# HorizonRobotics/HoloAgent

Hardware: AMD Instinct MI355X
Metric: HMSG frames/sec (one scene per GPU: map A1-A2, fusion A3-A5, merge A6, pooling A7, floors A8, rooms by the device watershed N1, room clouds, room embeddings and View nodes A9, objects with the view <-> object test A10 and graph assembly A11, nothing handed in -- plus 1000 coarse-to-fine retrieval qu (higher is better)
Workload: dtype f64 geometry / f32 features

## Files before the change

### holoagent_amd/csrc/hmsg_api.hip

```cpp
#include "hmsg_boundary.h"
#include "hmsg_ckdtree.h"
#include "hmsg_nn.h"
#include "hmsg_rle.h"

#include <algorithm>
#include <cstring>
#include <stdexcept>

void hmsg_bitset(hmsg_ctx* h, int first, int n, int M, const unsigned char* d_masks, const int* d_nmask);
void hmsg_fp_tables(hmsg_ctx* h, int first, int n, int M, const float* d_fg, const float* d_fm, const float* d_fc, const int* d_nmask);

__global__ void k_nn_patch(const long long* __restrict__ qid, const int* __restrict__ val, unsigned n, int* __restrict__ target) {
    const unsigned i = blockIdx.x * blockDim.x + threadIdx.x;
    if (i < n) target[qid[i]] = val[i];
}

void hmsg_kd_join(hmsg_ctx* h) {
    if (h->kd_thread.joinable()) h->kd_thread.join();
}

void hmsg_kd_start(hmsg_ctx* h) {
    hmsg_kd_join(h);
    h->host_pts.resize((size_t)h->V * 3);
    if (h->V) HIP_TRY(hipMemcpyAsync(h->host_pts.data(), h->pts.p, (size_t)h->V * 24, hipMemcpyDeviceToHost, h->stream));
// ... 129 lines not shown
        HIP_TRY(hipSetDevice(cfg->device_id));
        HIP_TRY(hipStreamCreateWithFlags(&h->stream, hipStreamNonBlocking));
        alloc_frame_store(h);
        h->pose.alloc((size_t)16 * cfg->max_frames);
    });
    if (rc != HMSG_OK) {
        delete h;
        return rc;
    }
    *out = h;
    return HMSG_OK;
}

void hmsg_destroy(hmsg_t* h) {
    if (!h) return;
    hmsg_kd_join(h);
    (void)hipSetDevice(h->cfg.device_id);
    try {
        hmsg_fold_pipe_abort(h);
    } catch (...) {
    }
    hmsg_graph_early_abort(h);
    h->fold_cache.trim();
    if (h->stream) {
        (void)hipStreamSynchronize(h->stream);
        (void)hipStreamDestroy(h->stream);
    }
    delete h;
}

const char* hmsg_last_error(const hmsg_t* h) { return h ? h->err.c_str() : "null handle"; }

void hmsg_release_cached_memory(void) { dev_cache().trim(); }

int hmsg_reset(hmsg_t* h) {
    if (!h) return HMSG_ERR_INVALID;
    return hmsg_boundary(h, [&] {
        HIP_TRY(hipStreamSynchronize(h->stream));
        hmsg_kd_join(h);
        hmsg_fold_pipe_abort(h);
        hmsg_graph_early_abort(h);
        ++h->inst_epoch;
        h->n_tie_queries = 0;
        h->n_frames = h->n_feat_frames = h->n_fused = 0;
        h->n_offered = 0;
        h->room_n = 0;
// ... 528 lines not shown
```

### holoagent_amd/csrc/hmsg_common.h

```cpp
#pragma once
#include <hip/hip_runtime.h>

#include <algorithm>
#include <chrono>
#include <cstdarg>
#include <cstdint>
#include <cstdio>
#include <cstdlib>
#include <cstring>
#include <map>
#include <memory>
#include <mutex>
#include <thread>
#include <string>
#include <vector>

#include "../../include/hmsg.h"
#include "../../include/hmsg_test.h"

#define HMSG_WAVE 64

struct hmsg_error {
    int code;
    std::string msg;
// ... 232 lines not shown
    ScopedEvent() { HIP_TRY(hipEventCreate(&e)); }
    ScopedEvent(const ScopedEvent&) = delete;
    ScopedEvent& operator=(const ScopedEvent&) = delete;
    ~ScopedEvent() { (void)hipEventDestroy(e); }
    operator hipEvent_t() const { return e; }
};

template <typename T>
struct PinnedBuf {
    T* p = nullptr;
    size_t n = 0;
    PinnedBuf() = default;
    PinnedBuf(const PinnedBuf&) = delete;
    PinnedBuf& operator=(const PinnedBuf&) = delete;
    ~PinnedBuf() {
        if (p) (void)hipHostFree(p);
    }
    void ensure(size_t count) {
        if (count <= n) return;
        if (p) (void)hipHostFree(p);
        p = nullptr;
        n = std::max<size_t>(count * 2, 256);
        HIP_TRY(hipHostMalloc((void**)&p, n * sizeof(T), hipHostMallocDefault));
    }
};
inline void d2h_bounce(void* dst, const void* src, size_t bytes) {
    constexpr size_t CH = (size_t)16 << 20;
    if (bytes <= 4096) {
        HIP_TRY(hipMemcpy(dst, src, bytes, hipMemcpyDeviceToHost));
        return;
    }
    static std::mutex mu;
    static PinnedBuf<unsigned char> stage;
    std::lock_guard<std::mutex> lk(mu);
    stage.ensure(std::min(bytes, CH));
    for (size_t o = 0; o < bytes; o += CH) {
        const size_t n = std::min(CH, bytes - o);
        HIP_TRY(hipMemcpy(stage.p, (const unsigned char*)src + o, n, hipMemcpyDeviceToHost));
        memcpy((unsigned char*)dst + o, stage.p, n);
    }
}
inline void h2d_bounce(void* dst_dev, const void* src_host, size_t bytes, hipStream_t s) {
    constexpr size_t CH = (size_t)16 << 20;
    if (!bytes) return;
    if (bytes <= 65536) {
        HIP_TRY(hipMemcpyAsync(dst_dev, src_host, bytes, hipMemcpyHostToDevice, s));
// ... 311 lines not shown
    bool merged = false;
    int frame_window = 0;
    bool tree_partial = false;
    long long merge_tree_batch = 0;
    bool frames_released = false;
    DevBuf<float> inst_feats;
    bool pooled = false;
    std::shared_ptr<struct FoldPipe> fold_pipe;
    int fold_pipe_frames = 0;
    DevCache fold_cache;
    bool restored = false;
    bool inst_denoised = false;
    struct hmsg_graph* early_graph = nullptr;
    unsigned long long inst_epoch = 0;
    int early_last = 0;
    std::shared_ptr<void> early_ops;
    std::vector<hmsg_node> nodes;
    DevBuf<int> room_sel, room_fmap;
    DevBuf<long long> room_off_dev;
    std::shared_ptr<void> room_scratch;
    int room_n = 0;
    long long room_total = 0;
    std::vector<int> node_label;
    DevBuf<unsigned> scan_tmp;
};

__device__ __forceinline__ unsigned long long scan_pack(unsigned epoch, unsigned flag, unsigned value) {
    return ((unsigned long long)((epoch << 2) | flag) << 32) | (unsigned long long)value;
}
__device__ __forceinline__ unsigned scan_lookback_prefix(unsigned long long* __restrict__ state, long long tile, unsigned epoch,
                                                         unsigned agg) {
    const int lane = threadIdx.x & 63;
    if (lane == 0)
        __hip_atomic_store(&state[tile], scan_pack(epoch, tile == 0 ? 2u : 1u, agg), __ATOMIC_RELAXED, __HIP_MEMORY_SCOPE_AGENT);
    unsigned prefix = 0;
    if (tile > 0) {
        long long hi = tile - 1;
        for (;;) {
            const long long idx = hi - lane;
            unsigned long long sw = scan_pack(epoch, 2u, 0u);
            if (idx >= 0) sw = __hip_atomic_load(&state[idx], __ATOMIC_RELAXED, __HIP_MEMORY_SCOPE_AGENT);
            const unsigned tag = (unsigned)(sw >> 32);
            const unsigned flag = (tag >> 2) == (epoch & 0x3fffffffu) ? (tag & 3u) : 0u;
            const unsigned long long has_prefix = __ballot(flag == 2u), not_ready = __ballot(flag == 0u);
            unsigned long long take = ~0ull;
            if (has_prefix) {
// ... 100 lines not shown
```

### holoagent_amd/csrc/hmsg_graph.hip

```cpp
#include "hmsg_boundary.h"
#include "hmsg_nn.h"
#include "hmsg_view_project.h"
#include <chrono>
#include "hmsg_ckdtree.h"

#include <cmath>

void hmsg_node_labels(hmsg_ctx* h, int n_labels, const float* label_feats) {
    const int N = (int)h->inst.off.size() - 1, D = h->cfg.feat_dim;
    h->node_label.assign((size_t)std::max(N, 0), -1);
    if (N <= 0 || n_labels <= 0) return;
    hmsg_index_t* ix = nullptr;
    std::vector<int32_t> zero((size_t)n_labels, 0);
    HMSG_REQUIRE(hmsg_index_create(h->cfg.device_id, D, n_labels, label_feats, 0, zero.data(), &ix) == HMSG_OK, HMSG_ERR_HIP,
                 "hmsg_build_object_nodes: label table");
    std::vector<double> S((size_t)N * n_labels);
    int rc = hmsg_similarity(ix, N, h->inst_feats.p, S.data());
    hmsg_index_destroy(ix);
    HMSG_REQUIRE(rc == HMSG_OK, HMSG_ERR_HIP, "hmsg_build_object_nodes: label similarity");
    for (int i = 0; i < N; ++i) {
        int best = 0;
        for (int l = 1; l < n_labels; ++l)
            if (S[(size_t)i * n_labels + l] > S[(size_t)i * n_labels + best]) best = l;
        h->node_label[(size_t)i] = best;
    }
}

void hmsg_object_nodes_on(hipStream_t s, const InstanceSet& inst, int n_floors, const double* floor_zero, const double* floor_height, int n_rooms,
                          const int32_t* room_floor, const int64_t* vert_off, const double* verts_xz, const double* share,
                          std::vector<hmsg_node>& nodes) {
    const int N = (int)inst.off.size() - 1;
    nodes.clear();
    std::vector<double> rc((size_t)n_rooms * 2, 0.0);
    for (int r = 0; r < n_rooms; ++r) {
        double sx = 0.0, sz = 0.0;
        for (long long v = vert_off[r]; v < vert_off[r + 1]; ++v) {
            sx += verts_xz[v * 2];
            sz += verts_xz[v * 2 + 1];
        }
        const double n = (double)(vert_off[r + 1] - vert_off[r]);
        rc[(size_t)r * 2] = sx / n;
// ... 615 lines not shown
```

### holoagent_amd/csrc/hmsg_query.h

```cpp
#pragma once
#include "hmsg_common.h"

typedef double f64x4 __attribute__((ext_vector_type(4)));

struct hmsg_index {
    int device = 0;
    int D = 0;
    long long N = 0;
    int n_rooms = 0;
    hipStream_t stream = nullptr;
    std::string err;
    DevBuf<double> E;
    DevBuf<int> room_of;
    DevBuf<int> room_off;
    DevBuf<int> room_nodes;
    std::vector<int> h_room_cnt;
    DevBuf<double> T64, S;
    DevBuf<float> Tf;
    DevBuf<int> d_qid, d_roff, d_rooms, d_oidx, d_oroom;
    DevBuf<double> d_oscore;
    bool have_hier = false;
    int n_floors = 0, h_rooms = 0;
    long long n_views = 0;
    DevBuf<double> room_name_emb;
// ... 11 lines not shown
    DevBuf<char> d_qout;
    long long n_obj_views = -1;
    std::vector<long long> h_vo_off;
    DevBuf<long long> vo_off;
    DevBuf<int> vo_nodes;
    DevBuf<int> d_view, d_vnode;
    DevBuf<double> d_vscore;
    Prof prof;
};

__device__ __forceinline__ f64x4 gemm_f64_tile16(const double* __restrict__ ap, bool a_ok, const double* __restrict__ bp, bool b_ok, int D) {
    f64x4 acc = {0.0, 0.0, 0.0, 0.0};
    const int kq = (threadIdx.x & 63) >> 4;
    for (int k0 = 0; k0 < D; k0 += 4) {
        const int k = k0 + kq;
        const double a = (k < D && a_ok) ? ap[k] : 0.0;
        const double b = (k < D && b_ok) ? bp[k] : 0.0;
        acc = __builtin_amdgcn_mfma_f64_16x16x4f64(a, b, acc, 0, 0, 0);
    }
    return acc;
}
void hmsg_gemm_f64(const double* A, int M, const double* B, long long N, int D, double* S, hipStream_t s);
hmsg_index* hmsg_index_create_rooms_only(int device, int D);


struct QueryScan {
    bool need_label = false, need_view = false;
    bool in_range = true;
    int max_floor = -1;
};
QueryScan hmsg_query_scan(int Q, const int* room_mode, const int* floor_id);
std::string hmsg_query_precondition(const char* who, const QueryScan& sc, int n_floors, bool have_room_text, bool have_room_names);
void hmsg_text_rows_to_f64(hipStream_t s, const float* src, size_t n, DevBuf<float>& tmp, DevBuf<double>& dst);
bool hmsg_query_pack_words(int* h_words, int Q, const int* floor_id, const int* room_mode, const int* qid);
struct QueryOut {
    int Q, k, max_rooms;
    size_t o_sel, o_nsel, o_err, o_idx, o_room, bytes;
    QueryOut(int Q_, int k_, int max_rooms_)
        : Q(Q_), k(k_), max_rooms(max_rooms_), o_sel((size_t)Q_ * k_ * 8), o_nsel(o_sel + (size_t)Q_ * max_rooms_ * 4), o_err(o_nsel + (size_t)Q_ * 4),
          o_idx(o_err + (size_t)Q_ * 4), o_room(o_idx + (size_t)Q_ * k_ * 4), bytes(o_room + (size_t)Q_ * k_ * 4) {}
    double* score(char* base) const { return (double*)base; }
    int* sel(char* base) const { return (int*)(base + o_sel); }
    int* nsel(char* base) const { return (int*)(base + o_nsel); }
    int* err(char* base) const { return (int*)(base + o_err); }
    int* idx(char* base) const { return (int*)(base + o_idx); }
    int* room(char* base) const { return (int*)(base + o_room); }
// ... 4 lines not shown
```

### holoagent_amd/csrc/hmsg_query.hip

```cpp
#include "hmsg_boundary.h"
#include "hmsg_query_rules.h"

#include <algorithm>
#include <chrono>

__global__ void k_f32_to_f64(const float* __restrict__ a, double* __restrict__ b, size_t n) {
    size_t i = (size_t)blockIdx.x * blockDim.x + threadIdx.x;
    if (i < n) b[i] = (double)a[i];
}

__global__ void __launch_bounds__(256) k_gemm_f64(const double* __restrict__ A, const double* __restrict__ B, int M, long long N,
                                                  int D, double* __restrict__ S) {
    const int lane = threadIdx.x & 63, wv = threadIdx.x >> 6;
    const long long tn = (N + 15) / 16;
    long long tile = (long long)blockIdx.x * 4 + wv;
    const long long ntiles = (long long)((M + 15) / 16) * tn;
    const bool active = tile < ntiles;
    if (!active) tile = ntiles - 1;
    const int m0 = (int)(tile / tn) * 16;
    const long long n0 = (tile % tn) * 16;
    const int ar = m0 + (lane & 15);
    const long long br = n0 + (lane & 15);
    const double* ap = A + (size_t)(ar < M ? ar : M - 1) * D;
    const double* bp = B + (size_t)(br < N ? br : N - 1) * D;
    const f64x4 acc = gemm_f64_tile16(ap, ar < M, bp, br < N, D);
    if (!active) return;
    const long long col = n0 + (lane & 15);
// ... 131 lines not shown
                                                     const double* __restrict__ S_view, long long n_views,
                                                     const int* __restrict__ view_off, const int* __restrict__ room_key,
                                                     const int* __restrict__ floor_room_off, const int* __restrict__ floor_rooms,
                                                     const int* __restrict__ floor_id, const int* __restrict__ mode, int max_sel,
                                                     int* __restrict__ sel, int* __restrict__ nsel, int* __restrict__ q_rooms,
                                                     int* __restrict__ err) {
    const int q = blockIdx.x, f = floor_id[q];
    IndexRooms src;
    src.S_room = S_room + (size_t)q * n_rooms;
    src.S_view = S_view + (size_t)q * n_views;
    src.view_off = view_off;
    src.keys = room_key;
    src.bad_floor = f >= n_floors;
    src.list = f < 0 || src.bad_floor ? nullptr : floor_rooms + floor_room_off[f];
    src.L = f < 0 ? n_rooms : (src.bad_floor ? 0 : floor_room_off[f + 1] - floor_room_off[f]);
    room_select(src, mode[q], max_sel, sel + (size_t)q * max_sel, nsel + q, q_rooms + (size_t)q * max_sel, err + q);
}
__global__ void k_fill_offsets(int* off, int n, int stride) {
    const int i = blockIdx.x * blockDim.x + threadIdx.x;
    if (i <= n) off[i] = i * stride;
}

namespace {
void gemm(hmsg_index* ix, const double* A, int M, double* S, const double* B = nullptr, long long N = -1) {
    if (!B) {
        B = ix->E.p;
        N = ix->N;
    }
    if (M >= 64 && N >= 64) {
        ProfScope ps(ix->prof, ix->stream, "k_gemm_f64", 2.0 * (double)M * (double)N * (double)ix->D);
        hmsg_gemm_f64(A, M, B, N, ix->D, S, ix->stream);
        return;
    }
    hmsg_gemm_f64(A, M, B, N, ix->D, S, ix->stream);
}
}

void hmsg_gemm_f64(const double* A, int M, const double* B, long long N, int D, double* S, hipStream_t s) {
    if (M <= 0 || N <= 0) return;
    if (M >= 64 && N >= 64) {
        const long long tiles = (long long)((M + GT - 1) / GT) * ((N + GT - 1) / GT);
        hipLaunchKernelGGL(k_gemm_f64_tiled, dim3((unsigned)tiles), dim3(256), 0, s, A, B, M, N, D, S);
    } else {
        const long long tiles = (long long)((M + 15) / 16) * ((N + 15) / 16);
        hipLaunchKernelGGL(k_gemm_f64, dim3(cdiv((size_t)tiles, 4)), dim3(256), 0, s, A, B, M, N, D, S);
    }
    HMSG_CHECK_LAUNCH();
}

hmsg_index* hmsg_index_create_rooms_only(int device, int D) {
    hmsg_index* ix = new hmsg_index();
    ix->device = device;
    ix->D = D;
    try {
        HIP_TRY(hipSetDevice(device));
        HIP_TRY(hipStreamCreateWithFlags(&ix->stream, hipStreamNonBlocking));
        ix->room_off.alloc(1);
        const int zero = 0;
        HIP_TRY(hipMemcpy(ix->room_off.p, &zero, 4, hipMemcpyHostToDevice));
    } catch (...) {
        hmsg_index_destroy(ix);
        throw;
    }
    return ix;
}

QueryScan hmsg_query_scan(int Q, const int* room_mode, const int* floor_id) {
    QueryScan sc;
    for (int q = 0; q < Q; ++q) {
        sc.in_range = sc.in_range && room_mode[q] >= 0 && room_mode[q] <= 3 && floor_id[q] >= -1;
        sc.need_label |= room_mode[q] == 1;
        sc.need_view |= room_mode[q] >= 2;
        sc.max_floor = std::max(sc.max_floor, floor_id[q]);
    }
    return sc;
}
std::string hmsg_query_precondition(const char* who, const QueryScan& sc, int n_floors, bool have_room_text, bool have_room_names) {
    const std::string w = std::string(who) + ": ";
    if (!sc.in_range || (n_floors >= 0 && sc.max_floor >= n_floors)) return w + "bad floor id / room mode";
// ... 31 lines not shown
    one(out_idx, o_idx, (size_t)Q * k * 4);
    one(out_room, o_room, (size_t)Q * k * 4);
    if (any_dev) HIP_TRY(hipStreamSynchronize(s));
    const int* herr = (const int*)(h + o_err);
    for (int q = 0; q < Q; ++q)
        HMSG_REQUIRE(!herr[q], HMSG_ERR_INVALID,
                     std::string(who) + ": a query's room stage failed like the reference would (a room without view embeddings, or a "
                                        "view-mode room number that is no position of the floor's room list)");
}

extern "C" {

int hmsg_index_create(int32_t device_id, int32_t dim, int64_t n, const void* emb, int32_t emb_is_f64, const int32_t* room_of_node,
                      hmsg_index_t** out) {
    if (!out) return HMSG_ERR_INVALID;
    *out = nullptr;
    if (dim <= 0 || n <= 0 || !emb || !room_of_node) return HMSG_ERR_INVALID;
    hmsg_index* ix = nullptr;
    const int rc = hmsg_boundary("hmsg_index_create", device_id, [&] {
        ix = new hmsg_index();
        ix->device = device_id;
        ix->D = dim;
        ix->N = n;
        HIP_TRY(hipStreamCreateWithFlags(&ix->stream, hipStreamNonBlocking));
        ix->E.alloc((size_t)n * dim);
        const size_t cnt = (size_t)n * dim;
        if (emb_is_f64) {
            copy_in(ix->E.p, emb, cnt * 8, ix->stream, Up::bounce);
        } else {
            DevBuf<float> tmp;
            const float* e32 = stage_in(tmp, (const float*)emb, cnt, ix->stream, Up::bounce);
            hipLaunchKernelGGL(k_f32_to_f64, dim3(cdiv(cnt, 256)), dim3(256), 0, ix->stream, e32, ix->E.p, cnt);
            HMSG_CHECK_LAUNCH();
            HIP_TRY(hipStreamSynchronize(ix->stream));
        }
        std::vector<int> rooms((size_t)n);
        read_in(rooms.data(), room_of_node, (size_t)n * 4);
        int nr = 0;
        for (int r : rooms) {
            HMSG_REQUIRE(r >= 0, HMSG_ERR_INVALID, "negative room id");
            nr = std::max(nr, r + 1);
        }
        ix->n_rooms = nr;
        std::vector<int> off(nr + 1, 0), nodes((size_t)n);
        for (int r : rooms) off[r + 1]++;
        for (int r = 0; r < nr; ++r) off[r + 1] += off[r];
        std::vector<int> cur(off.begin(), off.end() - 1);
        for (long long i = 0; i < n; ++i) nodes[cur[rooms[i]]++] = (int)i;
        ix->room_of.alloc((size_t)n);
        ix->room_off.alloc(nr + 1);
        ix->room_nodes.alloc((size_t)n);
        HIP_TRY(hipMemcpyAsync(ix->room_of.p, rooms.data(), (size_t)n * 4, hipMemcpyHostToDevice, ix->stream));
        HIP_TRY(hipMemcpyAsync(ix->room_off.p, off.data(), (size_t)(nr + 1) * 4, hipMemcpyHostToDevice, ix->stream));
        HIP_TRY(hipMemcpyAsync(ix->room_nodes.p, nodes.data(), (size_t)n * 4, hipMemcpyHostToDevice, ix->stream));
        HIP_TRY(hipStreamSynchronize(ix->stream));
    });
    if (rc != HMSG_OK) {
        delete ix;
        return rc;
    }
    *out = ix;
    return HMSG_OK;
}

void hmsg_index_destroy(hmsg_index_t* ix) {
    if (!ix) return;
    (void)hipSetDevice(ix->device);
    if (ix->stream) {
        (void)hipStreamSynchronize(ix->stream);
        (void)hipStreamDestroy(ix->stream);
    }
    ix->prof.clear();
    delete ix;
}

const char* hmsg_index_last_error(const hmsg_index_t* ix) { return ix ? ix->err.c_str() : "null index"; }

int hmsg_index_set_profiling(hmsg_index_t* ix, int32_t on) {
    if (!ix) return HMSG_ERR_INVALID;
    ix->prof.enabled = on != 0;
    return HMSG_OK;
}
int hmsg_index_profile(hmsg_index_t* ix, int64_t* launches, double* total_ms, double* total_flop) {
    if (!ix || !launches || !total_ms || !total_flop) return HMSG_ERR_INVALID;
    (void)hipStreamSynchronize(ix->stream);
    *launches = 0;
    *total_ms = *total_flop = 0.0;
    for (auto& e : ix->prof.ev) {
        float t = 0.f;
        if (hipEventElapsedTime(&t, e.a, e.b) != hipSuccess) continue;
        ++*launches;
        *total_ms += t;
        *total_flop += e.work;
// ... 19 lines not shown
        HMSG_REQUIRE(nr == 0 || rooms, HMSG_ERR_INVALID, "rooms list missing");
        ix->d_qid.ensure(Q);
        ix->d_roff.ensure(Q + 1);
        ix->d_rooms.ensure(std::max(nr, 1));
        ix->d_oidx.ensure((size_t)Q * k);
        ix->d_oroom.ensure((size_t)Q * k);
        ix->d_oscore.ensure((size_t)Q * k);
        copy_in(ix->d_qid.p, qid, (size_t)Q * 4, ix->stream, Up::direct);
        HIP_TRY(hipMemcpyAsync(ix->d_roff.p, hoff.data(), (size_t)(Q + 1) * 4, hipMemcpyHostToDevice, ix->stream));
        copy_in(ix->d_rooms.p, rooms, (size_t)nr * 4, ix->stream, Up::direct);
        hipLaunchKernelGGL(k_query_topk, dim3(Q), dim3(256), 0, ix->stream, (const double*)ix->S.p, ix->N, C, (const int*)ix->d_qid.p,
                           (const int*)ix->d_roff.p, (const int*)ix->d_rooms.p, (const int*)ix->room_off.p,
                           (const int*)ix->room_nodes.p, ix->n_rooms, k, use_negatives, ix->d_oidx.p, ix->d_oroom.p, ix->d_oscore.p);
        HMSG_CHECK_LAUNCH();
        HIP_TRY(hipMemcpyAsync(out_idx, ix->d_oidx.p, (size_t)Q * k * 4, hipMemcpyDeviceToHost, ix->stream));
        HIP_TRY(hipMemcpyAsync(out_room, ix->d_oroom.p, (size_t)Q * k * 4, hipMemcpyDeviceToHost, ix->stream));
        HIP_TRY(hipMemcpyAsync(out_score, ix->d_oscore.p, (size_t)Q * k * 8, hipMemcpyDeviceToHost, ix->stream));
        HIP_TRY(hipStreamSynchronize(ix->stream));
    });
}

int hmsg_index_set_hierarchy(hmsg_index_t* ix, int32_t n_rooms, int32_t n_floors, const int32_t* floor_room_off, const int32_t* floor_rooms,
                             const double* room_name_emb, const int64_t* view_off, const double* view_emb, const int32_t* room_key) {
    if (!ix) return HMSG_ERR_INVALID;
    return hmsg_boundary(ix, [&] {
        const int R = n_rooms;
        HMSG_REQUIRE(R >= ix->n_rooms && n_floors >= 0 && (n_floors == 0 || (floor_room_off && floor_rooms)) && view_off && room_key,
                     HMSG_ERR_INVALID, "hmsg_index_set_hierarchy: bad argument");
        ix->h_rooms = R;
        for (int f = 0; f < n_floors; ++f)
            for (int j = floor_room_off[f]; j < floor_room_off[f + 1]; ++j)
                HMSG_REQUIRE(floor_rooms[j] >= 0 && floor_rooms[j] < R, HMSG_ERR_INVALID, "hmsg_index_set_hierarchy: room id out of range");
        const long long NV = view_off[R];
        HMSG_REQUIRE(NV >= 0 && NV < (1ll << 31) && (NV == 0 || view_emb), HMSG_ERR_INVALID, "hmsg_index_set_hierarchy: bad view table");
        ix->n_floors = n_floors;
        ix->n_views = NV;
        std::vector<int> voff((size_t)R + 1);
        for (int r = 0; r <= R; ++r) voff[(size_t)r] = (int)view_off[r];
        ix->view_off.alloc((size_t)R + 1);
        ix->room_key.alloc((size_t)std::max(R, 1));
        ix->floor_room_off.alloc((size_t)n_floors + 1);
        const int nfr = n_floors ? floor_room_off[n_floors] : 0;
        ix->floor_rooms.alloc((size_t)std::max(nfr, 1));
        HIP_TRY(hipMemcpyAsync(ix->view_off.p, voff.data(), ((size_t)R + 1) * 4, hipMemcpyHostToDevice, ix->stream));
        HIP_TRY(hipMemcpyAsync(ix->room_key.p, room_key, (size_t)R * 4, hipMemcpyHostToDevice, ix->stream));
        std::vector<int> zero(1, 0);
        HIP_TRY(hipMemcpyAsync(ix->floor_room_off.p, n_floors ? floor_room_off : zero.data(), ((size_t)n_floors + 1) * 4, hipMemcpyHostToDevice, ix->stream));
        if (nfr) HIP_TRY(hipMemcpyAsync(ix->floor_rooms.p, floor_rooms, (size_t)nfr * 4, hipMemcpyHostToDevice, ix->stream));
        if (room_name_emb) {
            ix->room_name_emb.alloc((size_t)std::max(R, 1) * ix->D);
            copy_in(ix->room_name_emb.p, room_name_emb, (size_t)R * ix->D * 8, ix->stream, Up::bounce);
        } else {
            ix->room_name_emb.release();
        }
        ix->view_emb.alloc((size_t)std::max<long long>(NV, 1) * ix->D);
        copy_in(ix->view_emb.p, view_emb, (size_t)NV * ix->D * 8, ix->stream, Up::bounce);
        HIP_TRY(hipStreamSynchronize(ix->stream));
        ix->have_hier = true;
    });
}

int hmsg_query_hier(hmsg_index_t* ix, int32_t Q, int32_t C, const float* T_obj, const int32_t* qid, const float* T_room,
                    const int32_t* floor_id, const int32_t* room_mode, int32_t k, int32_t use_negatives, int32_t max_rooms,
                    int32_t* out_sel, int32_t* out_nsel, int32_t* out_idx, int32_t* out_room, double* out_score) {
    if (!ix) return HMSG_ERR_INVALID;
    return hmsg_boundary(ix, [&] {
        HMSG_REQUIRE(ix->have_hier, HMSG_ERR_INVALID, "hmsg_query_hier: hmsg_index_set_hierarchy first");
        HMSG_REQUIRE(Q >= 0 && C >= 1 && T_obj && qid && floor_id && room_mode && k >= 1 && max_rooms >= 1 && out_sel && out_nsel && out_idx &&
                         out_room && out_score,
                     HMSG_ERR_INVALID, "hmsg_query_hier: bad argument");
        if (Q == 0) return;
        const int R = ix->h_rooms;
        static const bool dbg = getenv("HMSG_DEBUG_TIMING") != nullptr;
        auto t_prev = std::chrono::steady_clock::now();
        auto lap = [&](const char* what) {
            if (!dbg) return;
            (void)hipStreamSynchronize(ix->stream);
            const auto t = std::chrono::steady_clock::now();
            fprintf(stderr, "[hmsg query_hier] %-22s %.3f ms\n", what, std::chrono::duration<double, std::milli>(t - t_prev).count());
            t_prev = t;
        };
        const QueryScan sc = hmsg_query_scan(Q, room_mode, floor_id);
        const bool need_label = sc.need_label, need_view = sc.need_view;
// ... 64 lines not shown
```

### holoagent_amd/csrc/hmsg_scene_graph.hip

```cpp
#include "hmsg_boundary.h"
#include "hmsg_dbscan.h"
#include "hmsg_query.h"
#include "hmsg_query_views.h"
#include "hmsg_stage_files.h"

#include <dirent.h>
#include <sys/stat.h>

#include <algorithm>
#include <atomic>
#include <chrono>
#include <cmath>
#include <cstdio>
#include <map>
#include <memory>
#include <string>
#include <mutex>
#include <thread>
#include <vector>

namespace {

struct GFloor {
    std::string id, name;
// ... 90 lines not shown
    bool have_inv = false;
    std::vector<std::thread> workers;
    std::string worker_err;
    std::mutex worker_mu;
    bool begun = false, finished = false, loaded = false;
    bool merged = false;
    bool failed = false;
    double t_begin_ms = 0, t_finish_ms = 0, t_kmeans_wait_ms = 0;
    hmsg_index_t* ix = nullptr;
    hmsg_index_t* shard_ix = nullptr;
    hmsg_shard_ws* shard_ws = nullptr;
    hmsg_goal_table* goal = nullptr;
    std::vector<std::string> goal_bad;
    std::vector<std::vector<int>> view_lists;
    bool views_on_index = false;
    DevBuf<double> obj_pts;
    std::vector<long long> obj_pts_off;
    bool have_obj_pts = false;
    hipStream_t view_stream = nullptr;
    bool registered = false;
    std::unique_ptr<EarlyObjects> early;
    int early_state = HMSG_EARLY_NEVER_MADE;
    double t_early_ms = 0, t_early_wait_ms = 0;
    ~hmsg_graph() {
        if (registered && h) hmsg_graph_early_abort(h);
        for (auto& t : workers)
            if (t.joinable()) t.join();
        if (ix) hmsg_index_destroy(ix);
        if (shard_ix) hmsg_index_destroy(shard_ix);
        if (shard_ws) hmsg_shard_ws_free(shard_ws);
        if (goal) hmsg_goal_table_free(goal);
        if (view_stream) {
            (void)hipSetDevice(device);
            (void)hipStreamSynchronize(view_stream);
            (void)hipStreamDestroy(view_stream);
        }
    }
};

namespace {

void need(int rc, hmsg_ctx* h, const char* what) {
    if (rc != HMSG_OK) throw hmsg_error{rc, std::string(what) + ": " + (h ? hmsg_last_error(h) : "failed")};
}

std::string jstr(const std::string& s) {
    std::string o = "\"";
    char buf[16];
    for (size_t i = 0; i < s.size();) {
        const unsigned char c = (unsigned char)s[i];
        if (c == '"') o += "\\\"", ++i;
        else if (c == '\\') o += "\\\\", ++i;
        else if (c == '\n') o += "\\n", ++i;
        else if (c == '\r') o += "\\r", ++i;
        else if (c == '\t') o += "\\t", ++i;
        else if (c == '\b') o += "\\b", ++i;
        else if (c == '\f') o += "\\f", ++i;
        else if (c < 0x20) snprintf(buf, sizeof buf, "\\u%04x", c), o += buf, ++i;
        else if (c < 0x80) o += (char)c, ++i;
        else {
            unsigned cp = 0;
            int n = c >= 0xf0 ? 4 : (c >= 0xe0 ? 3 : 2);
            cp = c & (n == 4 ? 0x07 : (n == 3 ? 0x0f : 0x1f));
            for (int k = 1; k < n && i + k < s.size(); ++k) cp = (cp << 6) | ((unsigned char)s[i + k] & 0x3f);
            i += (size_t)n;
            if (cp >= 0x10000) {
                cp -= 0x10000;
// ... 262 lines not shown
            auto it = pos.find(oid);
            if (it != pos.end()) ks.insert(ks.end(), it->second.begin(), it->second.end());
        }
        std::sort(ks.begin(), ks.end());
        ks.erase(std::unique(ks.begin(), ks.end()), ks.end());
        v.objects = ks;
    }
    g->merged = true;
}

void join_workers(hmsg_graph* g) {
    const double t0 = now_ms();
    for (auto& t : g->workers)
        if (t.joinable()) t.join();
    g->workers.clear();
    g->t_kmeans_wait_ms += now_ms() - t0;
    if (!g->worker_err.empty()) throw hmsg_error{HMSG_ERR_INVALID, g->worker_err};
}

void build_view_lists(hmsg_graph* g) {
    std::map<std::string, int> obj_of_id;
    for (size_t k = 0; k < g->objects.size(); ++k) obj_of_id.emplace(g->objects[k].id, (int)k);
    g->view_lists.assign(g->views.size(), {});
    for (size_t v = 0; v < g->views.size(); ++v)
        for (auto& oid : g->views[v].object_ids) {
            auto it = obj_of_id.find(oid);
            if (it != obj_of_id.end()) g->view_lists[v].push_back(it->second);
        }
}

void make_views(const hmsg_graph* g, std::vector<GView>& views, std::vector<std::vector<int>>& room_views) {
    const int skip = std::max(1, g->prm.skip_frames);
    room_views.assign(g->rooms.size(), {});
    for (size_t fi = 0; fi < g->floors.size(); ++fi) {
        int view_index = 0;
        for (int ri : g->floors[fi].rooms) {
            const GRoom& rm = g->rooms[(size_t)ri];
            for (int img : rm.imgs) {
                GView v;
                v.id = g->floors[fi].id + "_" + std::to_string(rm.index_in_floor) + "_" + std::to_string(view_index++);
                v.floor = (int)fi;
                v.room_in_floor = rm.index_in_floor;
                v.img = (long long)img * skip;
                if (!g->img_paths.empty() && (size_t)img < g->img_paths.size()) {
                    v.img_path = g->img_paths[(size_t)img];
                    v.have_path = true;
// ... 174 lines not shown
        std::vector<int> pair_obj;
        for (size_t k = 0; k < g->objects.size(); ++k)
            for (int v : g->rooms[(size_t)g->objects[k].room].views) {
                pair_obj.push_back((int)k);
                pair_inst.push_back(g->objects[k].instance);
                pair_view.push_back(v);
            }
        if (!pair_obj.empty()) {
            const size_t NV = g->views.size();
            std::vector<double> pinv;
            std::vector<int32_t> wh;
            view_cameras(g, h, g->views, pinv, wh);
            HMSG_REQUIRE(h->have_K, HMSG_ERR_INVALID, "hmsg_graph_finish: no camera intrinsics (hmsg_add_frames)");
            std::vector<uint8_t> vis(pair_obj.size());
            std::vector<double> md(pair_obj.size());
            need(hmsg_object_views(h, (int32_t)NV, pinv.data(), wh.data(), h->K, (int64_t)pair_obj.size(), pair_inst.data(), pair_view.data(),
                                   g->prm.min_visible_ratio, g->prm.max_view_depth, vis.data(), md.data()),
                 h, "hmsg_object_views");
            laps.lap("hmsg_object_views");
            link_views(g, pair_obj, pair_view, vis, md);
        }
        laps.lap("view lists (host)");
    }
    for (auto& o : g->objects) {
        for (int v : o.views) o.view_ids.push_back(g->views[(size_t)v].id);
        if (o.best_view >= 0) o.best_view_id = g->views[(size_t)o.best_view].id, o.have_best = true;
    }
    for (auto& v : g->views)
        for (int k : v.objects) {
            v.object_ids.push_back(g->objects[(size_t)k].id);
            v.texts.push_back(g->objects[(size_t)k].name);
        }
    if (g->prm.merge_objects_graph && !g->objects.empty()) {
        std::vector<hmsg_node> nodes(g->objects.size());
        std::vector<float> node_emb(g->objects.size() * (size_t)g->D);
        need(hmsg_get_nodes(h, nodes.data(), node_emb.data()), h, "hmsg_get_nodes");
        graph_merge_objects(g, node_emb);
    }
    laps.lap("id / text lists (host)");
    std::vector<int32_t> obj_room, view_room(g->views.size(), -1), vobj;
    std::vector<int64_t> vooff(1, 0);
    std::vector<int32_t> room_floor;
    for (auto& rm : g->rooms) room_floor.push_back(rm.floor);
    for (auto& o : g->objects) obj_room.push_back(o.room);
    for (auto& v : g->views) {
        vobj.insert(vobj.end(), v.objects.begin(), v.objects.end());
        vooff.push_back((int64_t)vobj.size());
    }
    int64_t ne = 0;
    const int64_t cap = (int64_t)g->floors.size() + (int64_t)g->rooms.size() + (int64_t)g->objects.size() + (int64_t)g->views.size() + (int64_t)vobj.size() + 4;
    g->edges.assign((size_t)cap * 2, 0);
    if (hmsg_graph_edges((int32_t)g->floors.size(), (int32_t)g->rooms.size(), room_floor.data(), (int32_t)g->objects.size(), obj_room.data(),
                         (int32_t)g->views.size(), view_room.data(), vooff.data(), vobj.data(), (int64_t*)g->edges.data(), cap, &ne) != HMSG_OK)
        throw hmsg_error{HMSG_ERR_INVALID, "hmsg_graph_edges failed"};
    g->edges.resize((size_t)ne * 2);
    laps.lap("edges");
    build_view_lists(g);
    g->finished = true;
}

struct JVal {
    enum Kind { NUL, BOOL, NUM, STR, ARR, OBJ } kind = NUL;
// ... 512 lines not shown

int hmsg_graph_get_room_vertices(const hmsg_graph_t* g, int32_t room, double* xz, int64_t capacity) {
    if (!g || room < 0 || room >= (int32_t)g->rooms.size() || !xz) return HMSG_ERR_INVALID;
    const GRoom& rm = g->rooms[(size_t)room];
    if ((size_t)capacity < rm.verts.size()) return HMSG_ERR_INVALID;
    if (!rm.verts.empty()) memcpy(xz, rm.verts.data(), rm.verts.size() * 8);
    return HMSG_OK;
}

int hmsg_graph_get_room_embeddings(const hmsg_graph_t* g, int32_t room, float* emb, int64_t capacity) {
    if (!g || room < 0 || room >= (int32_t)g->rooms.size() || !emb) return HMSG_ERR_INVALID;
    const GRoom& rm = g->rooms[(size_t)room];
    const size_t n = (size_t)rm.n_emb * (size_t)g->D;
    if ((size_t)capacity < n) return HMSG_ERR_INVALID;
    if (g->loaded)
        for (size_t i = 0; i < n; ++i) emb[i] = (float)rm.emb64[i];
    else if (n) memcpy(emb, rm.emb.data(), n * 4);
    return HMSG_OK;
}

int hmsg_graph_to_json(const hmsg_graph_t* g, char* buf, int64_t capacity, int64_t* needed) {
    if (!g || !needed) return HMSG_ERR_INVALID;
    return hmsg_boundary(nullptr, -1, [&] {
        std::string s = "{\"floors\": [";
        for (size_t i = 0; i < g->floors.size(); ++i) {
            const GFloor& f = g->floors[i];
            if (i) s += ", ";
            std::vector<std::string> rids;
            for (int r : f.rooms) rids.push_back(g->rooms[(size_t)r].id);
            s += "{\"floor_id\": " + jstr(f.id) + ", \"name\": " + jstr(f.name) + ", \"rooms\": " + jlist(rids) + ", \"n_points\": " +
                 std::to_string((long long)(g->loaded ? (long long)(f.pts.size() / 3) : (long long)f.f.n_points)) + "}";
        }
        s += "], \"rooms\": [";
        for (size_t i = 0; i < g->rooms.size(); ++i) {
            const GRoom& r = g->rooms[i];
            if (i) s += ", ";
            std::vector<std::string> oids, vids;
            for (int o : r.objects) oids.push_back(g->objects[(size_t)o].id);
            if (g->loaded) vids = r.view_ids;
            else
                for (int v : r.views) vids.push_back(g->views[(size_t)v].id);
            s += "{\"room_id\": " + jstr(r.id) + ", \"name\": " + jstr(r.name) + ", \"floor_id\": " + jstr(g->floors[(size_t)r.floor].id) + ", \"objects\": " +
                 jlist(oids) + ", \"views\": " + jlist(vids) + ", \"represent_images\": [";
            for (size_t k = 0; k < r.represent.size(); ++k) s += (k ? ", " : "") + std::to_string(r.represent[k]);
            s += "], \"sample_images\": [";
            for (size_t k = 0; k < r.sample.size(); ++k) s += (k ? ", " : "") + std::to_string(r.sample[k]);
// ... 11 lines not shown
        s += "], \"objects\": [";
        for (size_t i = 0; i < g->objects.size(); ++i) {
            const GObject& o = g->objects[i];
            if (i) s += ", ";
            s += "{\"object_id\": " + jstr(o.id) + ", \"room_id\": " + jstr(o.room_id) + ", \"name\": " + jstr(o.name) + ", \"instance\": " +
                 std::to_string(o.instance) + ", \"label\": " + std::to_string(o.label) + ", \"view_ids\": " + jlist(o.view_ids) + ", \"best_view_id\": " +
                 (o.have_best ? jstr(o.best_view_id) : std::string("null")) + "}";
        }
        s += "], \"edges\": [";
        for (size_t i = 0; i + 1 < g->edges.size(); i += 2) s += (i ? ", [" : "[") + std::to_string(g->edges[i]) + ", " + std::to_string(g->edges[i + 1]) + "]";
        s += "]}";
        *needed = (int64_t)s.size() + 1;
        if (!buf) return;
        HMSG_REQUIRE(capacity >= *needed, HMSG_ERR_INVALID, "hmsg_graph_to_json: buf too small (see *needed)");
        memcpy(buf, s.c_str(), s.size() + 1);
    });
}

int hmsg_save(hmsg_graph_t* g, const char* dir) {
    if (!g || !dir) return HMSG_ERR_INVALID;
    return hmsg_boundary(&g->err, -1, [&] {
        HMSG_REQUIRE(g->finished && g->h, HMSG_ERR_INVALID, "hmsg_save: a graph built by hmsg_build_graph / hmsg_graph_finish (its clouds live in the scene handle)");
        hmsg_ctx* h = g->h;
        const std::string root = dir;
        for (const char* sub : {"floors", "rooms", "objects", "views"}) mkdirs(root + "/" + sub);
        const int64_t V = hmsg_map_size(h);
        std::vector<double> map((size_t)std::max<int64_t>(V, 1) * 3);
        if (V) need(hmsg_get_map_points(h, map.data(), nullptr), h, "hmsg_get_map_points");
        for (size_t fi = 0; fi < g->floors.size(); ++fi) {
            GFloor& fl = g->floors[fi];
            std::vector<double> slab;
            for (int64_t i = 0; i < V; ++i) {
                const double y = map[(size_t)i * 3 + 1];
                if (y >= fl.f.y_lo && y <= fl.f.y_hi) slab.insert(slab.end(), &map[(size_t)i * 3], &map[(size_t)i * 3 + 3]);
            }
            if (hmsg_write_ply((root + "/floors/" + fl.id + ".ply").c_str(), slab.data(), (int64_t)(slab.size() / 3)) != HMSG_OK)
                throw hmsg_error{HMSG_ERR_INVALID, "cannot write the floor cloud"};
            std::vector<std::string> rids;
            for (int r : fl.rooms) rids.push_back(g->rooms[(size_t)r].id);
            const std::string s_id = jstr(fl.id), s_name = jstr(fl.name), s_rooms = jlist(rids);
            double zeros[24] = {0};
            std::vector<hmsg_json_field> f = {raw("floor_id", s_id), raw("name", s_name), raw("rooms", s_rooms),
                                              hmsg_json_field{"vertices", HMSG_JSON_F64, 2, 8, 3, fl.have_verts ? &fl.verts[0][0] : zeros},
                                              num0("floor_height", &fl.f.height), num0("floor_zero_level", &fl.f.zero_level)};
            write_json_fields(root + "/floors/" + fl.id + ".json", f);
            for (int ri : fl.rooms) {
// ... 266 lines not shown
            room[k] = g->objects[k].room;
        }
        if (hmsg_index_create(g->device, D, (int64_t)g->objects.size(), emb.data(), 0, room.data(), &ix) != HMSG_OK)
            throw hmsg_error{HMSG_ERR_INVALID, "hmsg_index_create failed"};
    } else {
        std::vector<double> emb(g->objects.size() * (size_t)D);
        std::vector<int32_t> room(g->objects.size());
        for (size_t k = 0; k < g->objects.size(); ++k) {
            HMSG_REQUIRE((int)g->objects[k].emb.size() == D, HMSG_ERR_INVALID, "hmsg_graph_index: object " + g->objects[k].id + " was saved without an embedding");
            memcpy(&emb[k * (size_t)D], g->objects[k].emb.data(), (size_t)D * 8);
            room[k] = g->objects[k].room;
        }
        if (hmsg_index_create(g->device, D, (int64_t)g->objects.size(), emb.data(), 1, room.data(), &ix) != HMSG_OK)
            throw hmsg_error{HMSG_ERR_INVALID, "hmsg_index_create failed"};
    }
    const int R = (int)g->rooms.size();
    std::vector<int32_t> fro(1, 0), fr, key((size_t)R);
    for (auto& fl : g->floors) {
        for (int r : fl.rooms) fr.push_back(r);
        fro.push_back((int32_t)fr.size());
    }
    std::vector<int64_t> voff(1, 0);
    std::vector<double> vemb;
    for (int r = 0; r < R; ++r) {
        const GRoom& rm = g->rooms[(size_t)r];
        const size_t us = rm.id.rfind('_');
        key[(size_t)r] = atoi(rm.id.c_str() + (us == std::string::npos ? 0 : us + 1));
        if (g->loaded) vemb.insert(vemb.end(), rm.emb64.begin(), rm.emb64.end());
        else
            for (float x : rm.emb) vemb.push_back((double)x);
        voff.push_back(voff.back() + rm.n_emb);
    }
    const int rc = hmsg_index_set_hierarchy(ix, R, (int32_t)g->floors.size(), fro.data(), fr.data(), room_name_emb, voff.data(), vemb.empty() ? nullptr : vemb.data(),
                                            key.data());
    if (rc != HMSG_OK) {
        std::string e = hmsg_index_last_error(ix);
        hmsg_index_destroy(ix);
        throw hmsg_error{rc, "hmsg_index_set_hierarchy: " + e};
    }
    *out = ix;
}
}

extern "C" {

int hmsg_graph_index(hmsg_graph_t* g, const double* room_name_emb, hmsg_index_t** out) {
    if (!g || !out) return HMSG_ERR_INVALID;
    *out = nullptr;
    return hmsg_boundary(&g->err, -1, [&] { graph_make_index(g, room_name_emb, false, out); });
}

}

hmsg_index_t* hmsg_graph_shard_index(hmsg_graph* g, int* n_floor_rooms) {
    *n_floor_rooms = 0;
    for (auto& fl : g->floors) *n_floor_rooms += (int)fl.rooms.size();
    HMSG_REQUIRE(g->finished && !g->failed, HMSG_ERR_INVALID, "hmsg_graph_query_sharded: a graph built by hmsg_graph_finish or loaded by hmsg_load");
// ... 462 lines not shown
```

Measured before the change: 2830.

## Cache label index, pool index streams, defer id lists, upload f32 view embeddings

Keeps the label-similarity index on the scene handle, keyed by a content hash of the host label table, so repeated frames skip rebuilding it. Index streams and pinned buffers are recycled through a small global pool instead of being created and destroyed per index. Building the object/view id and text lists is deferred until JSON, save or merge actually needs them. Room view embeddings are uploaded as f32 and widened on the device rather than converted on the host. The label cache reuses state across calls, and the hash adds a host cost over the label table each frame.

```diff
diff --git a/holoagent_amd/csrc/hmsg_api.hip b/holoagent_amd/csrc/hmsg_api.hip
--- a/holoagent_amd/csrc/hmsg_api.hip
+++ b/holoagent_amd/csrc/hmsg_api.hip
@@ -175,6 +175,8 @@
     }
     hmsg_graph_early_abort(h);
     h->fold_cache.trim();
+    if (h->label_ix) hmsg_index_destroy(h->label_ix);
+    h->label_ix = nullptr;
     if (h->stream) {
         (void)hipStreamSynchronize(h->stream);
         (void)hipStreamDestroy(h->stream);
diff --git a/holoagent_amd/csrc/hmsg_common.h b/holoagent_amd/csrc/hmsg_common.h
--- a/holoagent_amd/csrc/hmsg_common.h
+++ b/holoagent_amd/csrc/hmsg_common.h
@@ -278,6 +278,10 @@
         p = nullptr;
         n = std::max<size_t>(count * 2, 256);
         HIP_TRY(hipHostMalloc((void**)&p, n * sizeof(T), hipHostMallocDefault));
+    }
+    void swap(PinnedBuf& o) {
+        std::swap(p, o.p);
+        std::swap(n, o.n);
     }
 };
 inline void d2h_bounce(void* dst, const void* src, size_t bytes) {
@@ -635,6 +639,9 @@
     int room_n = 0;
     long long room_total = 0;
     std::vector<int> node_label;
+    struct hmsg_index* label_ix = nullptr;
+    int label_ix_rows = 0;
+    unsigned long long label_ix_hash = 0;
     DevBuf<unsigned> scan_tmp;
 };
 
diff --git a/holoagent_amd/csrc/hmsg_graph.hip b/holoagent_amd/csrc/hmsg_graph.hip
--- a/holoagent_amd/csrc/hmsg_graph.hip
+++ b/holoagent_amd/csrc/hmsg_graph.hip
@@ -3,6 +3,7 @@
 #include "hmsg_view_project.h"
 #include <chrono>
 #include "hmsg_ckdtree.h"
+#include "hmsg_hash.h"
 
 #include <cmath>
 
@@ -10,13 +11,26 @@
     const int N = (int)h->inst.off.size() - 1, D = h->cfg.feat_dim;
     h->node_label.assign((size_t)std::max(N, 0), -1);
     if (N <= 0 || n_labels <= 0) return;
-    hmsg_index_t* ix = nullptr;
-    std::vector<int32_t> zero((size_t)n_labels, 0);
-    HMSG_REQUIRE(hmsg_index_create(h->cfg.device_id, D, n_labels, label_feats, 0, zero.data(), &ix) == HMSG_OK, HMSG_ERR_HIP,
-                 "hmsg_build_object_nodes: label table");
+    const bool keyed = !hmsg_is_device_ptr(label_feats);
+    const unsigned long long key = keyed ? hmsg_hash64(label_feats, (size_t)n_labels * D * sizeof(float)) : 0ull;
+    if (h->label_ix && !(keyed && h->label_ix_rows == n_labels && h->label_ix_hash == key)) {
+        hmsg_index_destroy(h->label_ix);
+        h->label_ix = nullptr;
+    }
+    hmsg_index_t* ix = h->label_ix;
+    if (!ix) {
+        std::vector<int32_t> zero((size_t)n_labels, 0);
+        HMSG_REQUIRE(hmsg_index_create(h->cfg.device_id, D, n_labels, label_feats, 0, zero.data(), &ix) == HMSG_OK, HMSG_ERR_HIP,
+                     "hmsg_build_object_nodes: label table");
+        if (keyed) {
+            h->label_ix = ix;
+            h->label_ix_rows = n_labels;
+            h->label_ix_hash = key;
+        }
+    }
     std::vector<double> S((size_t)N * n_labels);
     int rc = hmsg_similarity(ix, N, h->inst_feats.p, S.data());
-    hmsg_index_destroy(ix);
+    if (ix != h->label_ix) hmsg_index_destroy(ix);
     HMSG_REQUIRE(rc == HMSG_OK, HMSG_ERR_HIP, "hmsg_build_object_nodes: label similarity");
     for (int i = 0; i < N; ++i) {
         int best = 0;
diff --git a/holoagent_amd/csrc/hmsg_hash.h b/holoagent_amd/csrc/hmsg_hash.h
--- /dev/null
+++ b/holoagent_amd/csrc/hmsg_hash.h
@@ -0,0 +1,37 @@
+#pragma once
+#include <cstddef>
+#include <cstdint>
+#include <cstring>
+
+static inline uint64_t hmsg_hash_rotl(uint64_t x, int r) { return (x << r) | (x >> (64 - r)); }
+static inline uint64_t hmsg_hash_avalanche(uint64_t x) {
+    x ^= x >> 33;
+    x *= 0xff51afd7ed558ccdull;
+    x ^= x >> 33;
+    x *= 0xc4ceb9fe1a85ec53ull;
+    x ^= x >> 33;
+    return x;
+}
+static inline uint64_t hmsg_hash64(const void* data, size_t n) {
+    const unsigned char* p = (const unsigned char*)data;
+    const uint64_t K = 0x9e3779b97f4a7c15ull;
+    uint64_t h[4] = {0x243f6a8885a308d3ull, 0x13198a2e03707344ull, 0xa4093822299f31d0ull, 0x082efa98ec4e6c89ull};
+    size_t i = 0;
+    for (; i + 32 <= n; i += 32) {
+        uint64_t w[4];
+        memcpy(w, p + i, 32);
+        for (int l = 0; l < 4; ++l) h[l] = hmsg_hash_rotl((h[l] ^ w[l]) * K, 29);
+    }
+    int lane = 0;
+    for (; i + 8 <= n; i += 8, ++lane) {
+        uint64_t w;
+        memcpy(&w, p + i, 8);
+        h[lane] = hmsg_hash_rotl((h[lane] ^ w) * K, 29);
+    }
+    uint64_t tail = 0;
+    const size_t nt = n - i;
+    if (nt) memcpy(&tail, p + i, nt);
+    uint64_t x = hmsg_hash_avalanche(tail ^ ((uint64_t)nt << 56) ^ (uint64_t)n * K);
+    for (int l = 0; l < 4; ++l) x = hmsg_hash_avalanche(x ^ h[l]) + hmsg_hash_rotl(h[l], 17 + l);
+    return hmsg_hash_avalanche(x);
+}
diff --git a/holoagent_amd/csrc/hmsg_lazy.h b/holoagent_amd/csrc/hmsg_lazy.h
--- /dev/null
+++ b/holoagent_amd/csrc/hmsg_lazy.h
@@ -0,0 +1,18 @@
+#pragma once
+#include <atomic>
+#include <mutex>
+
+struct LazyOnce {
+    std::atomic<bool> made_{true};
+    std::mutex mu;
+    bool made() const { return made_.load(std::memory_order_acquire); }
+    void arm() { made_.store(false, std::memory_order_release); }
+    template <typename F>
+    void ensure(F&& make) {
+        if (made()) return;
+        std::lock_guard<std::mutex> lk(mu);
+        if (made()) return;
+        make();
+        made_.store(true, std::memory_order_release);
+    }
+};
diff --git a/holoagent_amd/csrc/hmsg_query.h b/holoagent_amd/csrc/hmsg_query.h
--- a/holoagent_amd/csrc/hmsg_query.h
+++ b/holoagent_amd/csrc/hmsg_query.h
@@ -57,6 +57,9 @@
 }
 void hmsg_gemm_f64(const double* A, int M, const double* B, long long N, int D, double* S, hipStream_t s);
 hmsg_index* hmsg_index_create_rooms_only(int device, int D);
+int hmsg_index_set_hierarchy_views(hmsg_index* ix, int32_t n_rooms, int32_t n_floors, const int32_t* floor_room_off, const int32_t* floor_rooms,
+                                   const double* room_name_emb, const int64_t* view_off, const void* view_emb, int view_emb_is_f32,
+                                   const int32_t* room_key);
 
 
 struct QueryScan {
diff --git a/holoagent_amd/csrc/hmsg_query.hip b/holoagent_amd/csrc/hmsg_query.hip
--- a/holoagent_amd/csrc/hmsg_query.hip
+++ b/holoagent_amd/csrc/hmsg_query.hip
@@ -3,6 +3,8 @@
 
 #include <algorithm>
 #include <chrono>
+#include <memory>
+#include <mutex>
 
 __global__ void k_f32_to_f64(const float* __restrict__ a, double* __restrict__ b, size_t n) {
     size_t i = (size_t)blockIdx.x * blockDim.x + threadIdx.x;
@@ -180,6 +182,49 @@
 }
 
 namespace {
+struct IndexShell {
+    int device = 0;
+    hipStream_t stream = nullptr;
+    PinnedBuf<int> h_qin;
+    PinnedBuf<char> h_qout;
+};
+constexpr size_t SHELLS_KEPT = 4, SHELL_PINNED_MAX = (size_t)32 << 20;
+std::mutex g_shell_mu;
+std::vector<std::unique_ptr<IndexShell>>& g_shells = *new std::vector<std::unique_ptr<IndexShell>>();
+
+void shell_take(hmsg_index* ix) {
+    {
+        std::lock_guard<std::mutex> lk(g_shell_mu);
+        for (size_t i = 0; i < g_shells.size(); ++i)
+            if (g_shells[i]->device == ix->device) {
+                ix->stream = g_shells[i]->stream;
+                ix->h_qin.swap(g_shells[i]->h_qin);
+                ix->h_qout.swap(g_shells[i]->h_qout);
+                g_shells.erase(g_shells.begin() + (long)i);
+                return;
+            }
+    }
+    HIP_TRY(hipStreamCreateWithFlags(&ix->stream, hipStreamNonBlocking));
+}
+void shell_give(hmsg_index* ix) {
+    if (!ix->stream) return;
+    if (ix->h_qin.n * sizeof(int) + ix->h_qout.n <= SHELL_PINNED_MAX) {
+        std::lock_guard<std::mutex> lk(g_shell_mu);
+        if (g_shells.size() < SHELLS_KEPT) {
+            std::unique_ptr<IndexShell> sh(new IndexShell());
+            sh->device = ix->device;
+            sh->stream = ix->stream;
+            sh->h_qin.swap(ix->h_qin);
+            sh->h_qout.swap(ix->h_qout);
+            g_shells.push_back(std::move(sh));
+            ix->stream = nullptr;
+            return;
+        }
+    }
+    (void)hipStreamDestroy(ix->stream);
+    ix->stream = nullptr;
+}
+
 void gemm(hmsg_index* ix, const double* A, int M, double* S, const double* B = nullptr, long long N = -1) {
     if (!B) {
         B = ix->E.p;
@@ -212,7 +257,7 @@
     ix->D = D;
     try {
         HIP_TRY(hipSetDevice(device));
-        HIP_TRY(hipStreamCreateWithFlags(&ix->stream, hipStreamNonBlocking));
+        shell_take(ix);
         ix->room_off.alloc(1);
         const int zero = 0;
         HIP_TRY(hipMemcpy(ix->room_off.p, &zero, 4, hipMemcpyHostToDevice));
@@ -290,7 +335,7 @@
         ix->device = device_id;
         ix->D = dim;
         ix->N = n;
-        HIP_TRY(hipStreamCreateWithFlags(&ix->stream, hipStreamNonBlocking));
+        shell_take(ix);
         ix->E.alloc((size_t)n * dim);
         const size_t cnt = (size_t)n * dim;
         if (emb_is_f64) {
@@ -324,7 +369,7 @@
         HIP_TRY(hipStreamSynchronize(ix->stream));
     });
     if (rc != HMSG_OK) {
-        delete ix;
+        hmsg_index_destroy(ix);
         return rc;
     }
     *out = ix;
@@ -336,7 +381,7 @@
     (void)hipSetDevice(ix->device);
     if (ix->stream) {
         (void)hipStreamSynchronize(ix->stream);
-        (void)hipStreamDestroy(ix->stream);
+        shell_give(ix);
     }
     ix->prof.clear();
     delete ix;
@@ -402,6 +447,14 @@
 
 int hmsg_index_set_hierarchy(hmsg_index_t* ix, int32_t n_rooms, int32_t n_floors, const int32_t* floor_room_off, const int32_t* floor_rooms,
                              const double* room_name_emb, const int64_t* view_off, const double* view_emb, const int32_t* room_key) {
+    return hmsg_index_set_hierarchy_views(ix, n_rooms, n_floors, floor_room_off, floor_rooms, room_name_emb, view_off, view_emb, 0, room_key);
+}
+
+}
+
+int hmsg_index_set_hierarchy_views(hmsg_index* ix, int32_t n_rooms, int32_t n_floors, const int32_t* floor_room_off, const int32_t* floor_rooms,
+                                   const double* room_name_emb, const int64_t* view_off, const void* view_emb, int view_emb_is_f32,
+                                   const int32_t* room_key) {
     if (!ix) return HMSG_ERR_INVALID;
     return hmsg_boundary(ix, [&] {
         const int R = n_rooms;
@@ -434,11 +487,21 @@
             ix->room_name_emb.release();
         }
         ix->view_emb.alloc((size_t)std::max<long long>(NV, 1) * ix->D);
-        copy_in(ix->view_emb.p, view_emb, (size_t)NV * ix->D * 8, ix->stream, Up::bounce);
+        DevBuf<float> v32;
+        const size_t nv = (size_t)NV * ix->D;
+        if (view_emb_is_f32 && nv) {
+            const float* e32 = stage_in(v32, (const float*)view_emb, nv, ix->stream, Up::bounce);
+            hipLaunchKernelGGL(k_f32_to_f64, dim3(cdiv(nv, 256)), dim3(256), 0, ix->stream, e32, ix->view_emb.p, nv);
+            HMSG_CHECK_LAUNCH();
+        } else {
+            copy_in(ix->view_emb.p, view_emb, nv * 8, ix->stream, Up::bounce);
+        }
         HIP_TRY(hipStreamSynchronize(ix->stream));
         ix->have_hier = true;
     });
 }
+
+extern "C" {
 
 int hmsg_query_hier(hmsg_index_t* ix, int32_t Q, int32_t C, const float* T_obj, const int32_t* qid, const float* T_room,
                     const int32_t* floor_id, const int32_t* room_mode, int32_t k, int32_t use_negatives, int32_t max_rooms,
diff --git a/holoagent_amd/csrc/hmsg_scene_graph.hip b/holoagent_amd/csrc/hmsg_scene_graph.hip
--- a/holoagent_amd/csrc/hmsg_scene_graph.hip
+++ b/holoagent_amd/csrc/hmsg_scene_graph.hip
@@ -1,5 +1,6 @@
 #include "hmsg_boundary.h"
 #include "hmsg_dbscan.h"
+#include "hmsg_lazy.h"
 #include "hmsg_query.h"
 #include "hmsg_query_views.h"
 #include "hmsg_stage_files.h"
@@ -136,6 +137,7 @@
     std::unique_ptr<EarlyObjects> early;
     int early_state = HMSG_EARLY_NEVER_MADE;
     double t_early_ms = 0, t_early_wait_ms = 0;
+    mutable LazyOnce lists;
     ~hmsg_graph() {
         if (registered && h) hmsg_graph_early_abort(h);
         for (auto& t : workers)
@@ -157,6 +159,27 @@
 void need(int rc, hmsg_ctx* h, const char* what) {
     if (rc != HMSG_OK) throw hmsg_error{rc, std::string(what) + ": " + (h ? hmsg_last_error(h) : "failed")};
 }
+
+const hmsg_graph* graph_lists(const hmsg_graph* cg) {
+    cg->lists.ensure([cg] {
+        hmsg_graph* g = const_cast<hmsg_graph*>(cg);
+        for (auto& o : g->objects) {
+            o.view_ids.clear();
+            for (int v : o.views) o.view_ids.push_back(g->views[(size_t)v].id);
+            if (o.best_view >= 0) o.best_view_id = g->views[(size_t)o.best_view].id, o.have_best = true;
+        }
+        for (auto& v : g->views) {
+            v.object_ids.clear();
+            v.texts.clear();
+            for (int k : v.objects) {
+                v.object_ids.push_back(g->objects[(size_t)k].id);
+                v.texts.push_back(g->objects[(size_t)k].name);
+            }
+        }
+    });
+    return cg;
+}
+hmsg_graph* graph_lists(hmsg_graph* g) { return const_cast<hmsg_graph*>(graph_lists((const hmsg_graph*)g)); }
 
 std::string jstr(const std::string& s) {
     std::string o = "\"";
@@ -465,6 +488,13 @@
     std::map<std::string, int> obj_of_id;
     for (size_t k = 0; k < g->objects.size(); ++k) obj_of_id.emplace(g->objects[k].id, (int)k);
     g->view_lists.assign(g->views.size(), {});
+    if (!g->lists.made()) {
+        std::vector<int> first(g->objects.size());
+        for (size_t k = 0; k < g->objects.size(); ++k) first[k] = obj_of_id.find(g->objects[k].id)->second;
+        for (size_t v = 0; v < g->views.size(); ++v)
+            for (int k : g->views[v].objects) g->view_lists[v].push_back(first[(size_t)k]);
+        return;
+    }
     for (size_t v = 0; v < g->views.size(); ++v)
         for (auto& oid : g->views[v].object_ids) {
             auto it = obj_of_id.find(oid);
@@ -685,22 +715,14 @@
         }
         laps.lap("view lists (host)");
     }
-    for (auto& o : g->objects) {
-        for (int v : o.views) o.view_ids.push_back(g->views[(size_t)v].id);
-        if (o.best_view >= 0) o.best_view_id = g->views[(size_t)o.best_view].id, o.have_best = true;
-    }
-    for (auto& v : g->views)
-        for (int k : v.objects) {
-            v.object_ids.push_back(g->objects[(size_t)k].id);
-            v.texts.push_back(g->objects[(size_t)k].name);
-        }
+    g->lists.arm();
     if (g->prm.merge_objects_graph && !g->objects.empty()) {
         std::vector<hmsg_node> nodes(g->objects.size());
         std::vector<float> node_emb(g->objects.size() * (size_t)g->D);
         need(hmsg_get_nodes(h, nodes.data(), node_emb.data()), h, "hmsg_get_nodes");
-        graph_merge_objects(g, node_emb);
-    }
-    laps.lap("id / text lists (host)");
+        graph_merge_objects(graph_lists(g), node_emb);
+    }
+    laps.lap("merge objects");
     std::vector<int32_t> obj_room, view_room(g->views.size(), -1), vobj;
     std::vector<int64_t> vooff(1, 0);
     std::vector<int32_t> room_floor;
@@ -1259,6 +1281,7 @@
 int hmsg_graph_to_json(const hmsg_graph_t* g, char* buf, int64_t capacity, int64_t* needed) {
     if (!g || !needed) return HMSG_ERR_INVALID;
     return hmsg_boundary(nullptr, -1, [&] {
+        graph_lists(g);
         std::string s = "{\"floors\": [";
         for (size_t i = 0; i < g->floors.size(); ++i) {
             const GFloor& f = g->floors[i];
@@ -1316,6 +1339,7 @@
     return hmsg_boundary(&g->err, -1, [&] {
         HMSG_REQUIRE(g->finished && g->h, HMSG_ERR_INVALID, "hmsg_save: a graph built by hmsg_build_graph / hmsg_graph_finish (its clouds live in the scene handle)");
         hmsg_ctx* h = g->h;
+        graph_lists(g);
         const std::string root = dir;
         for (const char* sub : {"floors", "rooms", "objects", "views"}) mkdirs(root + "/" + sub);
         const int64_t V = hmsg_map_size(h);
@@ -1628,17 +1652,18 @@
     }
     std::vector<int64_t> voff(1, 0);
     std::vector<double> vemb;
+    std::vector<float> vemb32;
     for (int r = 0; r < R; ++r) {
         const GRoom& rm = g->rooms[(size_t)r];
         const size_t us = rm.id.rfind('_');
         key[(size_t)r] = atoi(rm.id.c_str() + (us == std::string::npos ? 0 : us + 1));
         if (g->loaded) vemb.insert(vemb.end(), rm.emb64.begin(), rm.emb64.end());
-        else
-            for (float x : rm.emb) vemb.push_back((double)x);
+        else vemb32.insert(vemb32.end(), rm.emb.begin(), rm.emb.end());
         voff.push_back(voff.back() + rm.n_emb);
     }
-    const int rc = hmsg_index_set_hierarchy(ix, R, (int32_t)g->floors.size(), fro.data(), fr.data(), room_name_emb, voff.data(), vemb.empty() ? nullptr : vemb.data(),
-                                            key.data());
+    const void* views = g->loaded ? (vemb.empty() ? nullptr : (const void*)vemb.data()) : (vemb32.empty() ? nullptr : (const void*)vemb32.data());
+    const int rc = hmsg_index_set_hierarchy_views(ix, R, (int32_t)g->floors.size(), fro.data(), fr.data(), room_name_emb, voff.data(), views, g->loaded ? 0 : 1,
+                                                  key.data());
     if (rc != HMSG_OK) {
         std::string e = hmsg_index_last_error(ix);
         hmsg_index_destroy(ix);
```

New measurement: 2870 (median of 6 runs). Within noise of the previous version (+1.4%).
